# abarret/mp-block-preconditioners

Hardware: AMD Instinct MI355X
Metric: precond-applies/sec (higher is better)
Workload: dtype f64; 1 GPU; 1024x1024 MAC grid, approx-commutator Schur preconditioner apply (BASELINE configs[2]); n=1024, unknowns=5242880, inner_F=chebyshev:4, inner_P=chebyshev:4, parallelism=single, layout=sell, f_sweeps=matrix-free-march-auto, f_numerics=fast, d_g_gtg=matrix-free, gt_f_g=diamond-13, g_x_p=recomputed in the second F solve, launch=hipgraph

## Files before the change

mp-block-preconditioners_amd/csrc/mpbp.hip:

```cpp
#include <hip/hip_runtime.h>

#include <stdarg.h>
#include <stdint.h>
#include <stdio.h>
#include <string.h>

#include <type_traits>
#include <vector>

#include "mpbp.h"

namespace {

thread_local char g_err[1024] = "";
mpbp_kernel_opts g_defaults = {
     0,  1,  1,  0,  1,  512,  1,
     1,  1,  1,  2,  1,  1,
     65536,  1,  1,  1,  1,
     0,  1,  0,  1,  1, {0}};
thread_local const mpbp_kernel_opts* t_opts = nullptr;
inline const mpbp_kernel_opts& KO() { return t_opts ? *t_opts : g_defaults; }
struct OptsScope {
    const mpbp_kernel_opts* prev;
    explicit OptsScope(const mpbp_kernel_opts* o) : prev(t_opts) {
// ... 1652 lines not shown
        return (lr >= 0 && lr < L ? (f * L + lr) * n : ext_row(4, f, lr, L, oh, n)) + gc;
    }
    template <bool EDGE, class TA, class XA>
    __device__ double row(int f, int gr, int gc, const TA& ta, const XA& xa, double* fd, const Cell& cl) const;
    struct Stage { double face[2]; };
    __device__ Stage stage_pre(int gr, int gcw) const {
        const int32_t k = wrap(gr) * n + gcw;
        return {{uface[k], vface[k]}};
    }
    template <class TA>
    __device__ double stage_diag(int f, int gr, int gc, const TA& ta, const Stage& s) const;
};

template <int M>
struct FDiagCommon {
    __device__ static double dmul(const FStencilDev& P, double y) { return (M & 1) ? -y : P.d_u * y; }
    __device__ static double emul(const FStencilDev& P, int p, double y) {
        const bool eta1 = p ? (M & 4) != 0 : (M & 2) != 0;
        return eta1 ? y : (p ? P.eta_s : P.eta_n) * y;
    }
};
template <int M>
struct FDiagU : FDiagCommon<M> {
    double iph_jph, iph_jmh, xi_ii, fd;
    template <class TA>
    __device__ FDiagU(const FStencilDev& P, int p, const TA& ta, int gr, int gc, double th) {
        const double tij = ta.T(p, gr, gc - 1), tip1j = ta.T(p, gr, gc);
        const double tijp1 = ta.T(p, gr - 1, gc - 1), tip1jp1 = ta.T(p, gr - 1, gc);
        const double tijm1 = ta.T(p, gr + 1, gc - 1), tip1jm1 = ta.T(p, gr + 1, gc);
        iph_jph = 0.25 * (tij + tijp1 + tip1jp1 + tip1j);
        iph_jmh = 0.25 * (tij + tip1j + tijm1 + tip1jm1);
        const double iph_j = 0.5 * (tij + tip1j);
        xi_ii = xi_of(P.xi, iph_j);
        const double wt = p ? P.c * (1.0 - th) : P.c * th;
        const double Ldiag = P.idx2 * (-tip1j - tij) + P.idx2 * (-iph_jph - iph_jmh);
        fd = (wt - this->dmul(P, xi_ii)) + this->dmul(P, this->emul(P, p, Ldiag));
    }
};
template <int M>
struct FDiagV : FDiagCommon<M> {
    double tij, tijp1, imh_jph, iph_jph, xi_ii, fd;
    template <class TA>
    __device__ FDiagV(const FStencilDev& P, int p, const TA& ta, int gr, int gc, double th) {
        tij = ta.T(p, gr, gc);
        const double tip1j = ta.T(p, gr, gc + 1);
        tijp1 = ta.T(p, gr - 1, gc);
        const double tip1jp1 = ta.T(p, gr - 1, gc + 1);
        const double tim1j = ta.T(p, gr, gc - 1), tim1jp1 = ta.T(p, gr - 1, gc - 1);
        const double ip1_jph = 0.5 * (tij + tijp1);
        xi_ii = xi_of(P.xi, ip1_jph);
        const double wt = p ? P.c * (1.0 - th) : P.c * th;
        imh_jph = 0.25 * (tim1j + tim1jp1 + tij + tijp1);
        iph_jph = 0.25 * (tij + tip1j + tijp1 + tip1jp1);
        const double Ldiag = P.midy2 * (tijp1 + tij) - P.idx2 * (iph_jph + imh_jph);
        fd = (wt - this->dmul(P, xi_ii)) + this->dmul(P, this->emul(P, p, Ldiag));
    }
};

template <int M, class TA>
__device__ inline double f_stage_diag(const FStencilDev& P, int f, int gr, int gc, const TA& ta,
                                      const FStencilDev::Stage& s) {
    const int p = f >> 1;
    return (f & 1) == 0 ? FDiagU<M>(P, p, ta, gr, gc, s.face[0]).fd : FDiagV<M>(P, p, ta, gr, gc, s.face[1]).fd;
}
template <class TA>
__device__ inline double FStencilDev::stage_diag(int f, int gr, int gc, const TA& ta, const Stage& s) const {
    return f_stage_diag<0>(*this, f, gr, gc, ta, s);
}

template <bool EDGE, class TA, class XA, bool VIRT = false, int M = 0>
__device__ inline double f_row(const FStencilDev& P, int f, int gr, int gc, const TA& ta, const XA& xa,
                               double* fdiag, const double* face = nullptr) {
    const int n = P.n;
    const int p = f >> 1;
    const double idx2 = P.idx2;
    const double eta = p ? P.eta_s : P.eta_n;
    const bool eta1 = p ? (M & 4) != 0 : (M & 2) != 0;
    auto dmul = [&](double y) -> double { return (M & 1) ? -y : P.d_u * y; };
    auto emul = [&](double y) -> double { return eta1 ? y : eta * y; };
    auto sc = [&](double y) -> double {
        if constexpr ((M & 8) != 0) return eta1 ? idx2 * y : y * (p ? P.ce1 : P.ce0);
        else return emul(idx2 * y);
    };
    const int fu = 2 * p, fv = 2 * p + 1;
    const int32_t kc = VIRT ? P.wrap(gr) * n + P.wrap(gc) : gr * n + gc;
    auto T = [&](int r, int c) -> double { return ta.T(p, r, c); };
    const Wrap w{gr == 0, gr == n - 1, gc == 0, gc == n - 1};
    double acc = 0.0;
    const double xcross = xa.X(f ^ 2, gr, gc);
    if ((f & 1) == 0) {
        const double tij = T(gr, gc - 1), tip1j = T(gr, gc);
        const double th = face ? face[0] : P.uface[kc];
        const FDiagU<M> dd(P, p, ta, gr, gc, th);
        const double iph_jph = dd.iph_jph, iph_jmh = dd.iph_jmh, xi_ii = dd.xi_ii;
        const double fd = dd.fd;
        *fdiag = fd;
        const double lo[5] = {dmul(sc(iph_jph)) * xa.X(fu, gr - 1, gc),
                              dmul(sc(tij)) * xa.X(fu, gr, gc - 1),
                              fd * xa.X(fu, gr, gc),
                              dmul((M & 8) ? sc(tip1j) : emul(P.pow2 ? tip1j * idx2 : tip1j / P.dxdx)) * xa.X(fu, gr, gc + 1),
                              dmul(sc(iph_jmh)) * xa.X(fu, gr + 1, gc)};
        const double hi[4] = {dmul(sc(tij - iph_jph)) * xa.X(fv, gr, gc - 1),
                              dmul(sc(-tip1j + iph_jph)) * xa.X(fv, gr, gc),
                              dmul(sc(iph_jmh - tij)) * xa.X(fv, gr + 1, gc - 1),
                              dmul(sc(tip1j - iph_jmh)) * xa.X(fv, gr + 1, gc)};
        const double vcross = dmul(xi_ii);
        if (p == 1) acc += vcross * xcross;
        acc = add5<EDGE>(acc, lo, w);
        acc = add4<EDGE>(acc, hi, w.rl, w.c0);
        if (p == 0) acc += vcross * xcross;
    } else {
        const double th = face ? face[1] : P.vface[kc];
        const FDiagV<M> dd(P, p, ta, gr, gc, th);
        const double tij = dd.tij, tijp1 = dd.tijp1;
        const double imh_jph = dd.imh_jph, iph_jph = dd.iph_jph, xi_ii = dd.xi_ii;
        const double fd = dd.fd;
        *fdiag = fd;
        const double lo[4] = {dmul(sc(tijp1 - imh_jph)) * xa.X(fu, gr - 1, gc),
                              dmul(sc(iph_jph - tijp1)) * xa.X(fu, gr - 1, gc + 1),
                              dmul(sc(imh_jph - tij)) * xa.X(fu, gr, gc),
                              dmul(sc(tij - iph_jph)) * xa.X(fu, gr, gc + 1)};
        const double hi[5] = {dmul(sc(tijp1)) * xa.X(fv, gr - 1, gc),
                              dmul(sc(imh_jph)) * xa.X(fv, gr, gc - 1),
                              fd * xa.X(fv, gr, gc),
                              dmul(sc(iph_jph)) * xa.X(fv, gr, gc + 1),
                              dmul(sc(tij)) * xa.X(fv, gr + 1, gc)};
        const double vcross = dmul(xi_ii);
        if (p == 1) acc += vcross * xcross;
        acc = add4<EDGE>(acc, lo, w.r0, w.cl);
        acc = add5<EDGE>(acc, hi, w);
        if (p == 0) acc += vcross * xcross;
    }
    return acc;
}

__device__ inline double rcp_nr(double y) {
    double r = __builtin_amdgcn_rcp(y);
    double e = __builtin_fma(-y, r, 1.0);
    r = __builtin_fma(r, e, r);
    e = __builtin_fma(-y, r, 1.0);
    return __builtin_fma(r, e, r);
}
struct FStencilFast : FStencilDev {
    static constexpr bool kFast = true;
    struct Nb { double nw, nn, ne, w, c, e, sw, s; };
    template <class TA>
    __device__ static Nb nb(const TA& ta, int gr, int gc) {
        return {ta.T(0, gr - 1, gc - 1), ta.T(0, gr - 1, gc), ta.T(0, gr - 1, gc + 1), ta.T(0, gr, gc - 1),
                ta.T(0, gr, gc), ta.T(0, gr, gc + 1), ta.T(0, gr + 1, gc - 1), ta.T(0, gr + 1, gc)};
    }
    struct Co { double w, c, nn, kc, ks, ke, xu, xv; };
    __device__ Co coeffs(const Nb& t) const {
        const double wc = t.w + t.c;
        Co k;
        k.w = t.w; k.c = t.c; k.nn = t.nn;
        k.kc = 0.25 * ((t.nw + t.nn) + wc);
        k.ks = 0.25 * (wc + (t.sw + t.s));
        k.ke = 0.25 * ((t.nn + t.ne) + (t.c + t.e));
        const double hu = 0.5 * wc, hv = 0.5 * (t.nn + t.c);
        const double mx = -d_u * xi;
        k.xu = mx * (hu * (1.0 - hu));
        k.xv = mx * (hv * (1.0 - hv));
        return k;
    }
    __device__ double aco(int p) const { return d_u * (p ? eta_s : eta_n) * idx2; }
    struct W4 { double wu[2], wv[2]; };
    __device__ W4 weights(const Cell& cl) const {
        return {{c * cl.face[0], c * (1.0 - cl.face[0])}, {c * cl.face[1], c * (1.0 - cl.face[1])}};
    }
    template <class XA>
    __device__ void rows4_co(int gr, int gc, const Co& k, const W4& w, const XA& xa, double* acc) const {
        const double xdu = k.xu * (xa.X(0, gr, gc) - xa.X(2, gr, gc));
        const double xdv = k.xv * (xa.X(1, gr, gc) - xa.X(3, gr, gc));
#pragma unroll
        for (int p = 0; p < 2; ++p) {
            const int fu = 2 * p, fv = 2 * p + 1;
            auto ph = [&](double t) { return p ? 1.0 - t : t; };
            const double a = aco(p);
            const double A1 = ph(k.w), A2 = ph(k.c), B1 = ph(k.nn), KC = ph(k.kc), KS = ph(k.ks), KE = ph(k.ke);
            const double uC = xa.X(fu, gr, gc), uN = xa.X(fu, gr - 1, gc), uS = xa.X(fu, gr + 1, gc);
            const double uW = xa.X(fu, gr, gc - 1), uE = xa.X(fu, gr, gc + 1), uNE = xa.X(fu, gr - 1, gc + 1);
            const double vC = xa.X(fv, gr, gc), vN = xa.X(fv, gr - 1, gc), vS = xa.X(fv, gr + 1, gc);
            const double vW = xa.X(fv, gr, gc - 1), vE = xa.X(fv, gr, gc + 1), vSW = xa.X(fv, gr + 1, gc - 1);
            const double tn = (uN - uC) + (vC - vW), tc = (uE - uC) + (vS - vC);
            double br = KC * tn;
            br = __builtin_fma(A1, (uW - uC) + (vW - vSW), br);
            br = __builtin_fma(A2, tc, br);
            br = __builtin_fma(KS, (uS - uC) + (vSW - vS), br);
            acc[fu] = __builtin_fma(a, br, __builtin_fma(w.wu[p], uC, p ? -xdu : xdu));
            double bv = B1 * ((vN - vC) + (uN - uNE));
            bv = __builtin_fma(KC, -tn, bv);
            bv = __builtin_fma(KE, (vE - vC) + (uNE - uE), bv);
            bv = __builtin_fma(A2, tc, bv);
            acc[fv] = __builtin_fma(a, bv, __builtin_fma(w.wv[p], vC, p ? -xdv : xdv));
        }
    }
    template <bool RD = true, class TA, class XA>
    __device__ void rows4(int gr, int gc, const TA& ta, const XA& xa, const Cell& cl, double* acc, double* rd) const {
        const Co k = coeffs(nb(ta, gr, gc));
        const W4 w = weights(cl);
        rows4_co(gr, gc, k, w, xa, acc);
        if constexpr (RD) rdiag4_co(k, w, rd);
    }
    __device__ void rdiag4_co(const Co& k, const W4& w, double* rd) const {
#pragma unroll
        for (int p = 0; p < 2; ++p) {
            auto ph = [&](double t) { return p ? 1.0 - t : t; };
            const double a = aco(p);
            const double A1 = ph(k.w), A2 = ph(k.c), B1 = ph(k.nn), KC = ph(k.kc), KS = ph(k.ks), KE = ph(k.ke);
            rd[2 * p] = rcp_nr(__builtin_fma(-a, (A1 + A2) + (KC + KS), w.wu[p] + k.xu));
            rd[2 * p + 1] = rcp_nr(__builtin_fma(-a, (B1 + A2) + (KC + KE), w.wv[p] + k.xv));
        }
    }
    template <class TA>
    __device__ void rdiag4(int gr, int gc, const TA& ta, const Stage& sg, double* rd) const {
        const Co k = coeffs(nb(ta, gr, gc));
#pragma unroll
        for (int p = 0; p < 2; ++p) {
            auto ph = [&](double t) { return p ? 1.0 - t : t; };
            const double a = aco(p);
            const double A1 = ph(k.w), A2 = ph(k.c), B1 = ph(k.nn), KC = ph(k.kc), KS = ph(k.ks), KE = ph(k.ke);
            rd[2 * p] = rcp_nr(__builtin_fma(-a, (A1 + A2) + (KC + KS), c * ph(sg.face[0]) + k.xu));
            rd[2 * p + 1] = rcp_nr(__builtin_fma(-a, (B1 + A2) + (KC + KE), c * ph(sg.face[1]) + k.xv));
        }
    }
};

struct TGlob {
    const double* t;
    int n;
    __device__ double T(int sph, int r, int c) const {
        r = r < 0 ? r + n : (r >= n ? r - n : r);
        c = c < 0 ? c + n : (c >= n ? c - n : c);
        const double v = t[r * n + c];
        return sph ? 1.0 - v : v;
    }
};
template <bool CHEB>
__global__ void __launch_bounds__(256) k_f_fast_init(FStencilFast P, const double* __restrict__ b, double c2,
                                                     double* __restrict__ d, const double* __restrict__ sub,
                                                     double* __restrict__ xo) {
    const int64_t i = (int64_t)blockIdx.x * 256 + threadIdx.x;
    if (i >= (int64_t)P.L * P.n) return;
    const int lr = (int)(i / P.n), gc = (int)(i - (int64_t)lr * P.n);
    const int gr = P.r0 + lr;
    const int32_t k = gr * P.n + gc;
    const FStencilDev::Stage sg{{P.uface[k], P.vface[k]}};
    double rd[4];
    P.rdiag4(gr, gc, TGlob{P.cell, P.n}, sg, rd);
#pragma unroll
    for (int f = 0; f < 4; ++f) {
        const int64_t o = ((int64_t)f * P.L + lr) * P.n + gc;
        const double x0 = c2 * b[o] * rd[f];
        if constexpr (CHEB) d[o] = x0;
        xo[o] = sub ? sub[o] - x0 : x0;
    }
}

constexpr int kMB = 256;
constexpr int kMTileW = kMB + 2;
struct XRing {
    const double* x;
    int s[3];
    int gr, c0;
    __device__ double X(int f, int r, int c) const { return x[(f * 3 + s[r - gr + 1]) * kMTileW + (c - c0 + 1)]; }
};
template <int W, int OFF>
struct TRingT {
    const double* t;
    int s[3];
    int gr, c0;
    __device__ double T(int sph, int r, int c) const {
        const double v = t[s[r - gr + 1] * W + (c - c0 + OFF)];
        return sph ? 1.0 - v : v;
    }
};
using TRing = TRingT<kMTileW, 1>;

struct XPlain {
    const double* __restrict__ x;
    typedef double Raw;
    __device__ Raw load(int32_t i) const { return x[i]; }
    __device__ double value(const Raw& r) const { return r; }
    __device__ double operator()(int32_t i) const { return x[i]; }
};
struct XInitRaw {
    double b, d;
};
struct XInit {
    const double* __restrict__ b;
    const double* __restrict__ dg;
    double c2;
    typedef XInitRaw Raw;
    __device__ Raw load(int32_t i) const { return {b[i], dg[i]}; }
    __device__ double value(const Raw& r) const { return c2 * (r.b / r.d); }
    __device__ double operator()(int32_t i) const { return c2 * (b[i] / dg[i]); }
};

struct BNone {
    static constexpr bool on = false, part = false;
    struct Q {};
    __device__ Q load(int, int, int) const { return {}; }
    template <class TA>
    __device__ double b(int, int, int, int, const TA&, const Q&) const { return 0.0; }
};
template <bool PART>
struct GxBT {
    static constexpr bool on = true, part = PART;
    const double* __restrict__ xp;
    double d_p, inv, minv;
    int n;
    int L = 0, h = 0;
// ... 982 lines not shown
        for (int it = 0; it < IT; ++it) {
            const int i = tid + it * 256;
            if (i < PN) ps[i] = v[it];
        }
    }
    const int lr = tid >> 6, lc = tid & 63;
    int cr[NSL], cc[NSL], rr[NSL];
    bool own[NSL];
#pragma unroll
    for (int m = 0; m < NT; ++m) {
        cr[m] = r0 + lr + 4 * m; cc[m] = c0 + lc; own[m] = true; rr[m] = 0;
    }
#pragma unroll
    for (int r = 1; r <= H; ++r) {
        own[1 + r] = tid < 140 + 8 * r;
        rr[1 + r] = r;
        fs_ring_cell(r, own[1 + r] ? tid : 0, r0, c0, cr[1 + r], cc[1 + r]);
    }
    double fl[NSL][2], bl[BS::on ? 1 : NSL][4];
#pragma unroll
    for (int sl = 0; sl < NSL; ++sl) {
        if (!own[sl]) continue;
        const int gr = P.wrap(cr[sl]), gc = P.wrap(cc[sl]);
        const int32_t k = gr * n + gc;
        fl[sl][0] = P.uface[k];
        fl[sl][1] = P.vface[k];
        if constexpr (!BS::on) {
            const int br = in_row(cr[sl], P.h);
#pragma unroll
            for (int f = 0; f < 4; ++f) bl[sl][f] = a.b[(PART ? ext_row(4, f, br, P.L, P.h, n) : (f * n + br) * n) + gc];
        }
    }
    __syncthreads();
    const TTileT<T::TW> tt{ts, rbt, cbt};
    double d[NS][4], rd[NS][4], bv[NS][4], fc[NS][2];
#pragma unroll
    for (int sl = 0; sl < NSL; ++sl) {
        if (!own[sl]) continue;
        const int vr = cr[sl], vc = cc[sl];
        const int gr = P.wrap(vr), gc = P.wrap(vc);
        const FStencilDev::Stage sg{{fl[sl][0], fl[sl][1]}};
        double b4[4], r4[4];
        P.rdiag4(vr, vc, tt, sg, r4);
        if constexpr (BS::on) {
            const int pi = (vr - rb + 1) * PW + (vc - cb + 1);
            const typename BS::Q q{ps[pi], ps[pi - 1], ps[pi - PW]};
#pragma unroll
            for (int f = 0; f < 4; ++f) b4[f] = bs.b_at(f, vr, vc, gc == 0, gr == 0, tt, q);
        } else {
#pragma unroll
            for (int f = 0; f < 4; ++f) b4[f] = bl[sl][f];
        }
        const int si = (vr - rb) * T::RW + (vc - cb);
#pragma unroll
        for (int f = 0; f < 4; ++f) {
            const double x0 = a.c2_0 * b4[f] * r4[f];
            xa[f * T::N + si] = x0;
            if (sl < NS) {
                d[sl][f] = x0;
                rd[sl][f] = r4[f];
                bv[sl][f] = b4[f];
            }
        }
        if (sl < NS) {
            fc[sl][0] = sg.face[0];
            fc[sl][1] = sg.face[1];
        }
    }
    double* cur = xa;
    double* nxt = xb;
    double sv[NT][4];
#pragma unroll
    for (int l = 1; l <= H; ++l) {
        __syncthreads();
        const XTileT<T::RW, T::RH> xt{cur, rb, cb};
        const double c1 = a.c1[l - 1], c2 = a.c2[l - 1];
        if constexpr (SUB) {
            if (l == H) {
#pragma unroll
                for (int m = 0; m < NT; ++m) {
                    const int vr = cr[m], vc = cc[m];
                    if (vr >= hi || vc >= n) continue;
#pragma unroll
                    for (int f = 0; f < 4; ++f)
                        sv[m][f] = a.sub[PART ? P.out_row(f, vr - P.r0, vc) : f * nn + vr * n + vc];
                }
            }
        }
#pragma unroll
        for (int sl = 0; sl < NS; ++sl) {
            if (sl >= NT && (!own[sl] || rr[sl] > H - l)) continue;
            const int vr = cr[sl], vc = cc[sl];
            if (l == H && (vr >= hi || vc >= n)) continue;
            double acc[4], rdx[4];
            P.template rows4<false>(vr, vc, tt, xt, FStencilDev::Cell{{fc[sl][0], fc[sl][1]}}, acc, rdx);
            const int si = (vr - rb) * T::RW + (vc - cb);
#pragma unroll
            for (int f = 0; f < 4; ++f) {
                const double z = (bv[sl][f] - acc[f]) * rd[sl][f];
                const double dn = c1 * d[sl][f] + c2 * z;
                const double x = cur[f * T::N + si] + dn;
                if (l < H) {
                    nxt[f * T::N + si] = x;
                    d[sl][f] = dn;
                } else {
                    const int32_t o = PART ? P.out_row(f, vr - P.r0, vc) : f * nn + vr * n + vc;
                    if constexpr (SUB) a.x_out[o] = sv[sl < NT ? sl : 0][f] - x;
                    else a.x_out[o] = x;
                }
            }
        }
        double* t = cur;
        cur = nxt;
        nxt = t;
    }
}

template <int H>
inline bool fsolve_ok_n(int n) { return n >= FsTile<H>::TW && n >= FsTile<H>::TH; }
template <int H, bool PART, class BS>
int launch_fsolve_t(const FStencilFast& P, const FSolve& a, hipStream_t st, const BS& bs) {
    const int rows = PART ? P.L + 2 * P.ext : P.n;
    const int64_t tiles = (int64_t)((P.n + kFTW - 1) / kFTW) * ((rows + kFTH - 1) / kFTH);
    if (a.sub) k_fsolve<H, true, PART, BS><<<(unsigned)tiles, 256, 0, st>>>(P, a, bs);
    else k_fsolve<H, false, PART, BS><<<(unsigned)tiles, 256, 0, st>>>(P, a, bs);
    MPBP_HIP(hipGetLastError());
    return MPBP_OK;
}
template <int TW, int TH, int H>
struct FsGeom {
    static constexpr int RW = TW + 2 * H, RH = TH + 2 * H, N = RW * RH;
    static constexpr int TSW = RW + 2, TSH = RH + 2, TSN = TSW * TSH;
    static constexpr int NT = TW * TH / 256;
    static constexpr int ring(int r) { return 2 * TW + 2 * TH + 8 * r - 4; }
    static constexpr int q(int r) { return ring(r) / 4; }
    static constexpr int qa() {
        int s = 0;
        for (int r = 1; r < H; ++r) s += q(r);
        return s;
    }
};
template <int TW, int TH>
__device__ inline void fs_ring_cell_t(int r, int j, int r0, int c0, int& vr, int& vc) {
    const int w = TW + 2 * r;
    if (j < 2 * w) {
        vr = j < w ? r0 - r : r0 + TH - 1 + r;
        vc = c0 - r + (j < w ? j : j - w);
    } else {
        const int k = j - 2 * w;
        vr = r0 - r + 1 + (k >> 1);
        vc = (k & 1) ? c0 + TW - 1 + r : c0 - r;
    }
}
template <int TW, int TH, int H, bool SUB, bool PART, class BS>
__global__ void __launch_bounds__(256) __attribute__((amdgpu_waves_per_eu(2, 8))) MPBP_LDS_READS
k_fsolve_w(FStencilFast P, FSolve a, BS bs) {
    using T = FsGeom<TW, TH, H>;
    static_assert(TW * TH == 256 * T::NT && TW % 32 == 0, "whole rows of 32 lanes, NT cells per lane");
    static_assert((2 * TW + 2 * TH - 4) % 4 == 0, "every ring splits into four equal runs");
    static_assert(T::qa() <= 64 && T::q(H) <= 64, "one ring slot for rings 1 .. H - 1 and one for ring H");
    constexpr int NT = T::NT;
    constexpr int NSL = NT + 2;
    constexpr int NS = NT + 1;
    constexpr int PW = T::RW + 1, PN = PW * (T::RH + 1);
    constexpr int KW = T::RW + 1, KN = KW * (T::RH + 1);
    __shared__ double ts[T::TSN];
    __shared__ double kt[KN];
    __shared__ double xa[4 * T::N], xb[4 * T::N];
    __shared__ double ps[BS::on ? PN : 1];
    const int n = P.n, nn = n * n;
    const int tx = (n + TW - 1) / TW;
    const int bk = xcd_swizzle(blockIdx.x, gridDim.x);
    const int lo = PART ? P.r0 - P.ext : 0, hi = PART ? P.r0 + P.L + P.ext : n;
    const int r0 = lo + (bk / tx) * TH, c0 = (bk % tx) * TW;
    const int rbt = r0 - H - 1, cbt = c0 - H - 1, rb = r0 - H, cb = c0 - H;
    const int tid = threadIdx.x;
    auto in_row = [&](int vr, int h) {
        if constexpr (PART) {
            const int lr = vr - P.r0;
            return lr < -h ? -h : (lr >= P.L + h ? P.L + h - 1 : lr);
        } else {
            return P.wrap(vr);
        }
    };
    {
        constexpr int IT = (T::TSN + 255) / 256;
        double v[IT];
#pragma unroll
        for (int it = 0; it < IT; ++it) {
            const int i = tid + it * 256;
            if (i < T::TSN) {
                const int sr = i / T::TSW, sc = i - sr * T::TSW;
                v[it] = P.cell[P.wrap(rbt + sr) * n + P.wrap(cbt + sc)];
            }
        }
#pragma unroll
        for (int it = 0; it < IT; ++it) {
            const int i = tid + it * 256;
            if (i < T::TSN) ts[i] = v[it];
        }
    }
    if constexpr (BS::on) {
        constexpr int IT = (PN + 255) / 256;
        double v[IT];
#pragma unroll
        for (int it = 0; it < IT; ++it) {
            const int i = tid + it * 256;
            if (i < PN) {
                const int sr = i / PW, sc = i - sr * PW;
                const int pr = in_row(rb - 1 + sr, PART ? bs.h : 0);
                v[it] = bs.xp[(PART ? ext_row(1, 0, pr, P.L, bs.h, n) : pr * n) + P.wrap(cb - 1 + sc)];
            }
        }
#pragma unroll
        for (int it = 0; it < IT; ++it) {
            const int i = tid + it * 256;
            if (i < PN) ps[i] = v[it];
        }
    }
    const int lane = tid & 63, wv = tid >> 6;
    int cr[NSL], cc[NSL], rr[NSL];
    bool own[NSL];
#pragma unroll
    for (int m = 0; m < NT; ++m) {
        cr[m] = r0 + tid / TW + m * (256 / TW); cc[m] = c0 + tid % TW; own[m] = true; rr[m] = 0;
    }
    {
        int r = 0, j = 0, base = 0;
#pragma unroll
        for (int q = 1; q < H; ++q) {
            if (r == 0 && lane < base + T::q(q)) {
                r = q;
                j = wv * T::q(q) + lane - base;
            }
            base += T::q(q);
        }
        own[NT] = r != 0;
        rr[NT] = r;
        fs_ring_cell_t<TW, TH>(r ? r : 1, j, r0, c0, cr[NT], cc[NT]);
        own[NT + 1] = lane < T::q(H);
        rr[NT + 1] = H;
        fs_ring_cell_t<TW, TH>(H, own[NT + 1] ? wv * T::q(H) + lane : 0, r0, c0, cr[NT + 1], cc[NT + 1]);
    }
    double fl[NSL][2], bl[BS::on ? 1 : NSL][4];
#pragma unroll
    for (int sl = 0; sl < NSL; ++sl) {
        if (!own[sl]) continue;
        const int gr = P.wrap(cr[sl]), gc = P.wrap(cc[sl]);
        const int32_t k = gr * n + gc;
        fl[sl][0] = P.uface[k];
        fl[sl][1] = P.vface[k];
        if constexpr (!BS::on) {
            const int br = in_row(cr[sl], P.h);
#pragma unroll
            for (int f = 0; f < 4; ++f) bl[sl][f] = a.b[(PART ? ext_row(4, f, br, P.L, P.h, n) : (f * n + br) * n) + gc];
        }
    }
    __syncthreads();
    const TTileT<T::TSW> tt{ts, rbt, cbt};
    {
        constexpr int IK = (KN + 255) / 256;
#pragma unroll
        for (int it = 0; it < IK; ++it) {
            const int i = tid + it * 256;
            if (i < KN) {
                const int r = rb + i / KW, c = cb + i % KW;
                kt[i] = 0.25 * ((tt.T(0, r - 1, c - 1) + tt.T(0, r - 1, c)) + (tt.T(0, r, c - 1) + tt.T(0, r, c)));
            }
        }
    }
    double d[NS][4], rd[NS][4], bv[NS][4], kx[NS][2];
    typename FStencilFast::W4 wt[NS];
#pragma unroll
    for (int sl = 0; sl < NSL; ++sl) {
        if (!own[sl]) continue;
        const int vr = cr[sl], vc = cc[sl];
        const int gr = P.wrap(vr), gc = P.wrap(vc);
        const FStencilDev::Cell cl{{fl[sl][0], fl[sl][1]}};
        const typename FStencilFast::Co k = P.coeffs(P.nb(tt, vr, vc));
        const typename FStencilFast::W4 w = P.weights(cl);
        double b4[4], r4[4];
        P.rdiag4_co(k, w, r4);
        if constexpr (BS::on) {
            const int pi = (vr - rb + 1) * PW + (vc - cb + 1);
            const typename BS::Q q{ps[pi], ps[pi - 1], ps[pi - PW]};
#pragma unroll
            for (int f = 0; f < 4; ++f) b4[f] = bs.b_at(f, vr, vc, gc == 0, gr == 0, tt, q);
        } else {
#pragma unroll
            for (int f = 0; f < 4; ++f) b4[f] = bl[sl][f];
        }
        const int si = (vr - rb) * T::RW + (vc - cb);
#pragma unroll
        for (int f = 0; f < 4; ++f) {
            const double x0 = a.c2_0 * b4[f] * r4[f];
            xa[f * T::N + si] = x0;
            if (sl < NS) {
                d[sl][f] = x0;
                rd[sl][f] = r4[f];
                bv[sl][f] = b4[f];
            }
        }
        if (sl < NS) {
            kx[sl][0] = k.xu;
            kx[sl][1] = k.xv;
            wt[sl] = w;
        }
    }
    double* cur = xa;
    double* nxt = xb;
    double sv[NT][4];
#pragma unroll
    for (int l = 1; l <= H; ++l) {
        __syncthreads();
        const XTileT<T::RW, T::RH> xt{cur, rb, cb};
        const double c1 = a.c1[l - 1], c2 = a.c2[l - 1];
        if constexpr (SUB) {
            if (l == H) {
#pragma unroll
                for (int m = 0; m < NT; ++m) {
                    const int vr = cr[m], vc = cc[m];
                    if (vr >= hi || vc >= n) continue;
#pragma unroll
                    for (int f = 0; f < 4; ++f)
                        sv[m][f] = a.sub[PART ? P.out_row(f, vr - P.r0, vc) : f * nn + vr * n + vc];
                }
            }
        }
#pragma unroll
        for (int sl = 0; sl < NS; ++sl) {
            if (sl >= NT && (!own[sl] || rr[sl] > H - l)) continue;
            const int vr = cr[sl], vc = cc[sl];
            if (l == H && (vr >= hi || vc >= n)) continue;
            typename FStencilFast::Co k;
            k.w = tt.T(0, vr, vc - 1);
            k.c = tt.T(0, vr, vc);
            k.nn = tt.T(0, vr - 1, vc);
            const int ki = (vr - rb) * KW + (vc - cb);
            k.kc = kt[ki];
            k.ks = kt[ki + KW];
            k.ke = kt[ki + 1];
            k.xu = kx[sl][0];
            k.xv = kx[sl][1];
            double acc[4];
            P.rows4_co(vr, vc, k, wt[sl], xt, acc);
            const int si = (vr - rb) * T::RW + (vc - cb);
#pragma unroll
            for (int f = 0; f < 4; ++f) {
                const double z = (bv[sl][f] - acc[f]) * rd[sl][f];
                const double dn = c1 * d[sl][f] + c2 * z;
                if (l < H) {
                    nxt[f * T::N + si] = cur[f * T::N + si] + dn;
                    d[sl][f] = dn;
                } else {
                    const double x = cur[f * T::N + si] + dn;
                    const int32_t o = PART ? P.out_row(f, vr - P.r0, vc) : f * nn + vr * n + vc;
                    if constexpr (SUB) a.x_out[o] = sv[sl < NT ? sl : 0][f] - x;
                    else a.x_out[o] = x;
                }
            }
        }
        double* t = cur;
        cur = nxt;
        nxt = t;
    }
}
template <int TW, int TH, int H>
inline bool fsolve_w_ok_n(int n) { return n >= FsGeom<TW, TH, H>::TSW && n >= FsGeom<TW, TH, H>::TSH; }
template <int H, bool PART, class BS>
int launch_fsolve_w(const FStencilFast& P, const FSolve& a, hipStream_t st, const BS& bs) {
    constexpr int TW = 32, TH = 16;
    const int rows = PART ? P.L + 2 * P.ext : P.n;
    const int64_t tiles = (int64_t)((P.n + TW - 1) / TW) * ((rows + TH - 1) / TH);
    if (a.sub) k_fsolve_w<TW, TH, H, true, PART, BS><<<(unsigned)tiles, 256, 0, st>>>(P, a, bs);
    else k_fsolve_w<TW, TH, H, false, PART, BS><<<(unsigned)tiles, 256, 0, st>>>(P, a, bs);
    MPBP_HIP(hipGetLastError());
    return MPBP_OK;
}

inline bool fsolve_ok(int K, int n) { return (K == 3 && fsolve_ok_n<2>(n)) || (K == 4 && fsolve_ok_n<3>(n)); }
template <class BS = BNone>
int launch_fsolve(const FStencilDev& Pd, int K, const double* c1, const double* c2, const double* b, const double* sub,
                  double* x_out, hipStream_t st, const BS& bs = BS{}) {
    const FStencilFast P{Pd};
    const bool part = P.h != 0;
    int xp_h = 0;
    if constexpr (BS::on) {
        if (BS::part != part) return set_error(MPBP_ERR_ARG, "fsolve: G x_p's layout does not match F's");
        if constexpr (BS::part) xp_h = bs.h;
    }
    if (!fsolve_ok(K, P.n) || (!part && P.which != 0) ||
        (part && (P.which != 3 || P.h < P.ext + K - 1 || P.oh < P.ext || (BS::on && xp_h < P.ext + K))))
        return set_error(MPBP_ERR_ARG, "fsolve: one GPU whole grid, or owned + ext rows with b ext + K - 1 deep");
    if (!x_out || (!BS::on && !b) || x_out == b) return set_error(MPBP_ERR_ARG, "fsolve: bad vectors");
    FSolve a{b, sub, x_out, c2[0], {}, {}};
    for (int l = 1; l < K; ++l) {
        a.c1[l - 1] = c1[l];
        a.c2[l - 1] = c2[l];
    }
    constexpr bool bpart = BS::on && BS::part;
    if (KO().f_solve_tile) {
        if (!(K == 3 ? fsolve_w_ok_n<32, 16, 2>(P.n) : fsolve_w_ok_n<32, 16, 3>(P.n)))
            return set_error(MPBP_ERR_ARG, "fsolve: grid smaller than the 32 x 16 tile's staging");
        if constexpr (BS::on) {
            return K == 3 ? launch_fsolve_w<2, bpart>(P, a, st, bs) : launch_fsolve_w<3, bpart>(P, a, st, bs);
        } else {
            if (part) return K == 3 ? launch_fsolve_w<2, true>(P, a, st, bs) : launch_fsolve_w<3, true>(P, a, st, bs);
            return K == 3 ? launch_fsolve_w<2, false>(P, a, st, bs) : launch_fsolve_w<3, false>(P, a, st, bs);
        }
    }
    if constexpr (BS::on) {
        return K == 3 ? launch_fsolve_t<2, bpart>(P, a, st, bs) : launch_fsolve_t<3, bpart>(P, a, st, bs);
    } else {
        if (part) return K == 3 ? launch_fsolve_t<2, true>(P, a, st, bs) : launch_fsolve_t<3, true>(P, a, st, bs);
        return K == 3 ? launch_fsolve_t<2, false>(P, a, st, bs) : launch_fsolve_t<3, false>(P, a, st, bs);
    }
}

template <bool SUB, bool SD, class BS>
int launch_march2_t(const FStencilFast& P, const Fused2& a, hipStream_t st, const BS& bs) {
    const int64_t chunks = march_chunks(P, KO().march_rows, march_capacity<k_march2<SUB, SD, BS>>());
    if (chunks == 0) return MPBP_OK;
    const int64_t strips = (P.n + kMB - 1) / kMB;
    k_march2<SUB, SD, BS><<<(unsigned)(chunks * strips), kMB, 0, st>>>(P, a, (int)chunks, bs);
    MPBP_HIP(hipGetLastError());
    return MPBP_OK;
}
template <class BS = BNone>
int launch_march2(const FStencilDev& Pd, const Fused2& a, hipStream_t st, const BS& bs = BS{}) {
    const FStencilFast P{Pd};
    if (P.which == 1 || P.which == 2) return set_error(MPBP_ERR_ARG, "march2: interior / boundary row splits unsupported");
    if (!a.x_in || !a.d_in || !a.x_out || a.x_in == a.x_out || (!BS::on && !a.b) || (a.d_out && a.d_out == a.d_in))
        return set_error(MPBP_ERR_ARG, "march2: bad vectors");
    const bool sub = a.sub != nullptr, sd = a.d_out != nullptr;
    return sub ? (sd ? launch_march2_t<true, true>(P, a, st, bs) : launch_march2_t<true, false>(P, a, st, bs))
               : (sd ? launch_march2_t<false, true>(P, a, st, bs) : launch_march2_t<false, false>(P, a, st, bs));
}

template <class S, class Epi, class BS = BNone>
int launch_march_init(const S& P, const double* b, double c2, Epi epi, int rows_per_block, hipStream_t st,
                      const BS& bs = BS{}) {
    auto go = [&](const auto& e) {
        using E = std::decay_t<decltype(e)>;
        const int64_t chunks = march_chunks(P, rows_per_block, march_capacity<k_march_init<S, E, BS>>());
        if (chunks == 0) return (int)MPBP_OK;
        const int64_t strips = (P.n + kMB - 1) / kMB;
        k_march_init<S, E, BS><<<(unsigned)(chunks * strips), kMB, 0, st>>>(P, b, c2, (int)chunks, e, bs);
        MPBP_HIP(hipGetLastError());
        return (int)MPBP_OK;
    };
    if constexpr (BS::on) return with_fixed_epi_bx<S::kFast>(epi, go);
    else return with_fixed_epi<S::kFast>(epi, go);
}

template <class S, class XS, class Epi, class BS = BNone>
int launch_march(const S& P, const XS& xs, Epi epi, int rows_per_block, hipStream_t st, const BS& bs = BS{}) {
    auto go = [&](const auto& e) { return launch_march_fixed(P, xs, e, rows_per_block, st, bs); };
    if constexpr (BS::on) return with_fixed_epi_bx<S::kFast>(epi, go);
    else return with_fixed_epi<S::kFast>(epi, go);
}

template <bool EDGE, class TA, class XA>
__device__ inline double FStencilDev::row(int f, int gr, int gc, const TA& ta, const XA& xa, double* fd,
                                          const Cell& cl) const {
    return f_row<EDGE>(*this, f, gr, gc, ta, xa, fd, cl.face);
}

template <int M>
struct FStencilDevM : FStencilDev {
    template <bool EDGE, class TA, class XA>
    __device__ double row(int f, int gr, int gc, const TA& ta, const XA& xa, double* fd, const Cell& cl) const {
        return f_row<EDGE, TA, XA, false, M>(*this, f, gr, gc, ta, xa, fd, cl.face);
    }
    template <class TA>
    __device__ double stage_diag(int f, int gr, int gc, const TA& ta, const Stage& s) const {
        return f_stage_diag<M>(*this, f, gr, gc, ta, s);
    }
};

template <class Fn>
int with_f_identities(const FStencilDev& P, Fn&& fn);
template <class Fn>
int with_f_policy(const FStencilDev& P, bool fast, Fn&& fn) {
    if (fast) return fn(FStencilFast{P});
    return with_f_identities(P, fn);
}

template <class Fn>
int with_f_identities(const FStencilDev& P, Fn&& fn) {
    if (P.d_u == -1.0 && P.eta_s == 1.0) {
        if (P.eta_n != 1.0 && P.pow2 && P.ce0 != 0.0 && __builtin_isfinite(P.ce0)) return fn(FStencilDevM<13>{P});
        return P.eta_n == 1.0 ? fn(FStencilDevM<7>{P}) : fn(FStencilDevM<5>{P});
    }
    return fn(P);
}

struct PGDev {
    static constexpr bool kFast = false;
    int n;
    const double* cell;
    double d_p, inv, minv;
    int r0, L, h, which;
    int ext = 0;
    int oh = 0;
    int unit = 0;
    __device__ int wrap(int a) const { return a < 0 ? a + n : (a >= n ? a - n : a); }
    template <int NFI>
    __device__ int32_t xrow_of(int f, int gr) const {
        if (h == 0) return (f * n + wrap(gr)) * n;
        return ext_row(NFI, f, gr - r0, L, h, n);
    }
// ... 4629 lines not shown
```

Before: 6776 applies/s (1024^2-cell equivalents).

## Use tile-relative indexing and row-per-wave staging in the wavefront F-solve kernel

Reworks the fused Chebyshev F-solve kernel so each slot keeps tile-relative row and column offsets plus a precomputed global byte offset, replacing repeated wrap and global-index arithmetic. The cell, x_p and K-table staging now loads one tile row per wave, with lanes mapped to columns, which removes the integer divides. Stencil reads go through pointer-relative accessors to cut address math and register pressure. It adds an extra barrier after building the K table and assumes a staged row fits in one 64-lane wave.

```diff
diff --git a/mp-block-preconditioners_amd/csrc/mpbp.hip b/mp-block-preconditioners_amd/csrc/mpbp.hip
--- a/mp-block-preconditioners_amd/csrc/mpbp.hip
+++ b/mp-block-preconditioners_amd/csrc/mpbp.hip
@@ -1828,12 +1828,14 @@
     struct Co { double w, c, nn, kc, ks, ke, xu, xv; };
     __device__ Co coeffs(const Nb& t) const {
         const double wc = t.w + t.c;
+        return coeffs_k(t.w, t.c, t.nn, wc, 0.25 * ((t.nw + t.nn) + wc), 0.25 * (wc + (t.sw + t.s)),
+                        0.25 * ((t.nn + t.ne) + (t.c + t.e)));
+    }
+    __device__ Co coeffs_k(double w, double c, double nn, double wc, double kc, double ks, double ke) const {
         Co k;
-        k.w = t.w; k.c = t.c; k.nn = t.nn;
-        k.kc = 0.25 * ((t.nw + t.nn) + wc);
-        k.ks = 0.25 * (wc + (t.sw + t.s));
-        k.ke = 0.25 * ((t.nn + t.ne) + (t.c + t.e));
-        const double hu = 0.5 * wc, hv = 0.5 * (t.nn + t.c);
+        k.w = w; k.c = c; k.nn = nn;
+        k.kc = kc; k.ks = ks; k.ke = ke;
+        const double hu = 0.5 * wc, hv = 0.5 * (nn + c);
         const double mx = -d_u * xi;
         k.xu = mx * (hu * (1.0 - hu));
         k.xv = mx * (hv * (1.0 - hv));
@@ -3122,6 +3124,29 @@
         vc = (k & 1) ? c0 + TW - 1 + r : c0 - r;
     }
 }
+template <int TW, int TH>
+__device__ inline void fs_ring_rel(int r, int j, int h, int& dr, int& dc) {
+    const int w = TW + 2 * r, k = j - 2 * w;
+    const bool top = j < w, row = j < 2 * w;
+    dr = h + (row ? (top ? -r : TH - 1 + r) : 1 - r + (k >> 1));
+    dc = h + (row ? (top ? j : j - w) - r : ((k & 1) ? TW - 1 + r : -r));
+}
+template <class V>
+__device__ inline V* at_off(V* base, uint32_t off) { return (V*)((const char*)base + off); }
+__device__ inline double ld_off(const double* base, uint32_t off) { return *at_off(base, off); }
+template <int W>
+struct TRelT {
+    const double* t;
+    __device__ double T(int sph, int r, int c) const {
+        const double v = t[r * W + c];
+        return sph ? 1.0 - v : v;
+    }
+};
+template <int W, int N>
+struct XRelT {
+    const double* x;
+    __device__ double X(int f, int r, int c) const { return x[f * N + r * W + c]; }
+};
 template <int TW, int TH, int H, bool SUB, bool PART, class BS>
 __global__ void __launch_bounds__(256) __attribute__((amdgpu_waves_per_eu(2, 8))) MPBP_LDS_READS
 k_fsolve_w(FStencilFast P, FSolve a, BS bs) {
@@ -3132,8 +3157,9 @@
     constexpr int NT = T::NT;
     constexpr int NSL = NT + 2;
     constexpr int NS = NT + 1;
-    constexpr int PW = T::RW + 1, PN = PW * (T::RH + 1);
+    constexpr int PW = T::RW + 1, PH = T::RH + 1, PN = PW * PH;
     constexpr int KW = T::RW + 1, KN = KW * (T::RH + 1);
+    static_assert(T::TSW <= 64 && PW == KW, "a staged row is one wave's lanes; x_p's window and the K table share indices");
     __shared__ double ts[T::TSN];
     __shared__ double kt[KN];
     __shared__ double xa[4 * T::N], xb[4 * T::N];
@@ -3153,114 +3179,123 @@
             return P.wrap(vr);
         }
     };
+    const int lane = tid & 63, wv = __builtin_amdgcn_readfirstlane(tid >> 6) & 3;
+    const uint32_t gcs = 8u * (uint32_t)P.wrap(cbt + (lane < T::TSW ? lane : 0));
+    if (lane < T::TSW) {
+        constexpr int IT = (T::TSH + 3) / 4;
+        double v[IT];
+#pragma unroll
+        for (int it = 0; it < IT; ++it) {
+            const int sr = wv + 4 * it;
+            if (sr < T::TSH) v[it] = ld_off(P.cell + P.wrap(rbt + sr) * n, gcs);
+        }
+#pragma unroll
+        for (int it = 0; it < IT; ++it) {
+            const int sr = wv + 4 * it;
+            if (sr < T::TSH) ts[sr * T::TSW + lane] = v[it];
+        }
+    }
+    if constexpr (BS::on) {
+        if (lane < PW) {
+            constexpr int IT = (PH + 3) / 4;
+            double v[IT];
+#pragma unroll
+            for (int it = 0; it < IT; ++it) {
+                const int sr = wv + 4 * it;
+                if (sr < PH) {
+                    const int pr = in_row(rbt + sr, PART ? bs.h : 0);
+                    v[it] = ld_off(bs.xp + (PART ? ext_row(1, 0, pr, P.L, bs.h, n) : pr * n), gcs);
+                }
+            }
+#pragma unroll
+            for (int it = 0; it < IT; ++it) {
+                const int sr = wv + 4 * it;
+                if (sr < PH) ps[sr * PW + lane] = v[it];
+            }
+        }
+    }
+    int dr[NSL], dc[NSL];
+#pragma unroll
+    for (int m = 0; m < NT; ++m) {
+        dr[m] = H + tid / TW + m * (256 / TW); dc[m] = H + tid % TW;
+    }
+    int rA = 0;
+    dr[NT] = H; dc[NT] = H;
     {
-        constexpr int IT = (T::TSN + 255) / 256;
-        double v[IT];
-#pragma unroll
-        for (int it = 0; it < IT; ++it) {
-            const int i = tid + it * 256;
-            if (i < T::TSN) {
-                const int sr = i / T::TSW, sc = i - sr * T::TSW;
-                v[it] = P.cell[P.wrap(rbt + sr) * n + P.wrap(cbt + sc)];
-            }
-        }
-#pragma unroll
-        for (int it = 0; it < IT; ++it) {
-            const int i = tid + it * 256;
-            if (i < T::TSN) ts[i] = v[it];
-        }
-    }
-    if constexpr (BS::on) {
-        constexpr int IT = (PN + 255) / 256;
-        double v[IT];
-#pragma unroll
-        for (int it = 0; it < IT; ++it) {
-            const int i = tid + it * 256;
-            if (i < PN) {
-                const int sr = i / PW, sc = i - sr * PW;
-                const int pr = in_row(rb - 1 + sr, PART ? bs.h : 0);
-                v[it] = bs.xp[(PART ? ext_row(1, 0, pr, P.L, bs.h, n) : pr * n) + P.wrap(cb - 1 + sc)];
-            }
-        }
-#pragma unroll
-        for (int it = 0; it < IT; ++it) {
-            const int i = tid + it * 256;
-            if (i < PN) ps[i] = v[it];
-        }
-    }
-    const int lane = tid & 63, wv = tid >> 6;
-    int cr[NSL], cc[NSL], rr[NSL];
-    bool own[NSL];
-#pragma unroll
-    for (int m = 0; m < NT; ++m) {
-        cr[m] = r0 + tid / TW + m * (256 / TW); cc[m] = c0 + tid % TW; own[m] = true; rr[m] = 0;
-    }
-    {
-        int r = 0, j = 0, base = 0;
+        int base = 0;
 #pragma unroll
         for (int q = 1; q < H; ++q) {
-            if (r == 0 && lane < base + T::q(q)) {
-                r = q;
-                j = wv * T::q(q) + lane - base;
+            if (lane >= base && lane < base + T::q(q)) {
+                fs_ring_rel<TW, TH>(q, wv * T::q(q) + lane - base, H, dr[NT], dc[NT]);
+                rA = q;
             }
             base += T::q(q);
         }
-        own[NT] = r != 0;
-        rr[NT] = r;
-        fs_ring_cell_t<TW, TH>(r ? r : 1, j, r0, c0, cr[NT], cc[NT]);
-        own[NT + 1] = lane < T::q(H);
-        rr[NT + 1] = H;
-        fs_ring_cell_t<TW, TH>(H, own[NT + 1] ? wv * T::q(H) + lane : 0, r0, c0, cr[NT + 1], cc[NT + 1]);
-    }
+    }
+    const bool ownB = lane < T::q(H);
+    fs_ring_rel<TW, TH>(H, ownB ? wv * T::q(H) + lane : 0, H, dr[NT + 1], dc[NT + 1]);
+    auto own = [&](int sl) { return sl < NT || (sl == NT ? rA != 0 : ownB); };
     double fl[NSL][2], bl[BS::on ? 1 : NSL][4];
+    uint32_t kg[NSL];
+    bool ww[NSL], wn[NSL], outok[NT];
 #pragma unroll
     for (int sl = 0; sl < NSL; ++sl) {
-        if (!own[sl]) continue;
-        const int gr = P.wrap(cr[sl]), gc = P.wrap(cc[sl]);
-        const int32_t k = gr * n + gc;
-        fl[sl][0] = P.uface[k];
-        fl[sl][1] = P.vface[k];
+        if (!own(sl)) continue;
+        const int vr = rb + dr[sl], vc = cb + dc[sl];
+        const int gr = !PART && sl < NT ? (vr >= n ? vr - n : vr) : P.wrap(vr);
+        const int gc = sl < NT ? (vc >= n ? vc - n : vc) : P.wrap(vc);
+        kg[sl] = 8u * (uint32_t)(gr * n + gc);
+        ww[sl] = gc == 0;
+        wn[sl] = gr == 0;
+        if (sl < NT) outok[sl < NT ? sl : 0] = vr < hi && vc < n;
+        fl[sl][0] = ld_off(P.uface, kg[sl]);
+        fl[sl][1] = ld_off(P.vface, kg[sl]);
         if constexpr (!BS::on) {
-            const int br = in_row(cr[sl], P.h);
-#pragma unroll
-            for (int f = 0; f < 4; ++f) bl[sl][f] = a.b[(PART ? ext_row(4, f, br, P.L, P.h, n) : (f * n + br) * n) + gc];
+            if constexpr (PART) {
+                const int br = in_row(vr, P.h);
+#pragma unroll
+                for (int f = 0; f < 4; ++f) bl[sl][f] = a.b[ext_row(4, f, br, P.L, P.h, n) + gc];
+            } else {
+#pragma unroll
+                for (int f = 0; f < 4; ++f) bl[sl][f] = ld_off(a.b + (size_t)f * nn, kg[sl]);
+            }
         }
     }
     __syncthreads();
-    const TTileT<T::TSW> tt{ts, rbt, cbt};
-    {
-        constexpr int IK = (KN + 255) / 256;
+    if (lane < KW) {
+        constexpr int IK = (T::RH + 1 + 3) / 4;
 #pragma unroll
         for (int it = 0; it < IK; ++it) {
-            const int i = tid + it * 256;
-            if (i < KN) {
-                const int r = rb + i / KW, c = cb + i % KW;
-                kt[i] = 0.25 * ((tt.T(0, r - 1, c - 1) + tt.T(0, r - 1, c)) + (tt.T(0, r, c - 1) + tt.T(0, r, c)));
+            const int kr = wv + 4 * it;
+            if (kr < T::RH + 1) {
+                const double* t = ts + kr * T::TSW + lane;
+                kt[kr * KW + lane] = 0.25 * ((t[0] + t[1]) + (t[T::TSW] + t[T::TSW + 1]));
             }
         }
     }
+    __syncthreads();
     double d[NS][4], rd[NS][4], bv[NS][4], kx[NS][2];
     typename FStencilFast::W4 wt[NS];
 #pragma unroll
     for (int sl = 0; sl < NSL; ++sl) {
-        if (!own[sl]) continue;
-        const int vr = cr[sl], vc = cc[sl];
-        const int gr = P.wrap(vr), gc = P.wrap(vc);
+        if (!own(sl)) continue;
+        const int si = dr[sl] * T::RW + dc[sl], ki = si + dr[sl];
+        const double* t = ts + (ki + dr[sl] + T::TSW + 1);
         const FStencilDev::Cell cl{{fl[sl][0], fl[sl][1]}};
-        const typename FStencilFast::Co k = P.coeffs(P.nb(tt, vr, vc));
+        const double tw = t[-1], tc = t[0], tn = t[-T::TSW];
+        const typename FStencilFast::Co k = P.coeffs_k(tw, tc, tn, tw + tc, kt[ki], kt[ki + KW], kt[ki + 1]);
         const typename FStencilFast::W4 w = P.weights(cl);
         double b4[4], r4[4];
         P.rdiag4_co(k, w, r4);
         if constexpr (BS::on) {
-            const int pi = (vr - rb + 1) * PW + (vc - cb + 1);
+            const int pi = ki + PW + 1;
             const typename BS::Q q{ps[pi], ps[pi - 1], ps[pi - PW]};
 #pragma unroll
-            for (int f = 0; f < 4; ++f) b4[f] = bs.b_at(f, vr, vc, gc == 0, gr == 0, tt, q);
+            for (int f = 0; f < 4; ++f) b4[f] = bs.b_at(f, 0, 0, ww[sl], wn[sl], TRelT<T::TSW>{t}, q);
         } else {
 #pragma unroll
             for (int f = 0; f < 4; ++f) b4[f] = bl[sl][f];
         }
-        const int si = (vr - rb) * T::RW + (vc - cb);
 #pragma unroll
         for (int f = 0; f < 4; ++f) {
             const double x0 = a.c2_0 * b4[f] * r4[f];
@@ -3283,38 +3318,38 @@
 #pragma unroll
     for (int l = 1; l <= H; ++l) {
         __syncthreads();
-        const XTileT<T::RW, T::RH> xt{cur, rb, cb};
         const double c1 = a.c1[l - 1], c2 = a.c2[l - 1];
+        auto out_at = [&](auto* v, int m, int f) {
+            if constexpr (PART) return v + P.out_row(f, rb + dr[m] - P.r0, cb + dc[m]);
+            else return at_off(v + (size_t)f * nn, kg[m]);
+        };
         if constexpr (SUB) {
             if (l == H) {
 #pragma unroll
                 for (int m = 0; m < NT; ++m) {
-                    const int vr = cr[m], vc = cc[m];
-                    if (vr >= hi || vc >= n) continue;
-#pragma unroll
-                    for (int f = 0; f < 4; ++f)
-                        sv[m][f] = a.sub[PART ? P.out_row(f, vr - P.r0, vc) : f * nn + vr * n + vc];
+                    if (!outok[m]) continue;
+#pragma unroll
+                    for (int f = 0; f < 4; ++f) sv[m][f] = *out_at(a.sub, m, f);
                 }
             }
         }
 #pragma unroll
         for (int sl = 0; sl < NS; ++sl) {
-            if (sl >= NT && (!own[sl] || rr[sl] > H - l)) continue;
-            const int vr = cr[sl], vc = cc[sl];
-            if (l == H && (vr >= hi || vc >= n)) continue;
+            if (sl >= NT && (l == H || rA == 0 || rA > H - l)) continue;
+            if (l == H && !outok[sl < NT ? sl : 0]) continue;
+            const int si = dr[sl] * T::RW + dc[sl], ki = si + dr[sl];
+            const double* t = ts + (ki + dr[sl] + T::TSW + 1);
             typename FStencilFast::Co k;
-            k.w = tt.T(0, vr, vc - 1);
-            k.c = tt.T(0, vr, vc);
-            k.nn = tt.T(0, vr - 1, vc);
-            const int ki = (vr - rb) * KW + (vc - cb);
+            k.w = t[-1];
+            k.c = t[0];
+            k.nn = t[-T::TSW];
             k.kc = kt[ki];
             k.ks = kt[ki + KW];
             k.ke = kt[ki + 1];
             k.xu = kx[sl][0];
             k.xv = kx[sl][1];
             double acc[4];
-            P.rows4_co(vr, vc, k, wt[sl], xt, acc);
-            const int si = (vr - rb) * T::RW + (vc - cb);
+            P.rows4_co(0, 0, k, wt[sl], XRelT<T::RW, T::N>{cur + si}, acc);
 #pragma unroll
             for (int f = 0; f < 4; ++f) {
                 const double z = (bv[sl][f] - acc[f]) * rd[sl][f];
@@ -3324,9 +3359,8 @@
                     d[sl][f] = dn;
                 } else {
                     const double x = cur[f * T::N + si] + dn;
-                    const int32_t o = PART ? P.out_row(f, vr - P.r0, vc) : f * nn + vr * n + vc;
-                    if constexpr (SUB) a.x_out[o] = sv[sl < NT ? sl : 0][f] - x;
-                    else a.x_out[o] = x;
+                    if constexpr (SUB) *out_at(a.x_out, sl < NT ? sl : 0, f) = sv[sl < NT ? sl : 0][f] - x;
+                    else *out_at(a.x_out, sl < NT ? sl : 0, f) = x;
                 }
             }
         }
```

New measurement: 7023 applies/s (1024^2-cell equivalents), median of 6. 3.6% higher.
